# John-Ragland/pygenray

Measured on AMD Instinct MI355X. Metric: ray-steps/sec (whole node), 1e5-ray Munk fan to 1000 km; eigenray wall-clock, higher is better.
Workload: dtype f64

## Files before the change

pygenray_amd/csrc/pgr_crmath.h:

```cpp
#ifndef PGR_CRMATH_H
#define PGR_CRMATH_H

#ifdef PGR_CR_HOST
#include <math.h>
#define PGR_CR_FN static inline
#define PGR_CR_RARE(c) (__builtin_expect((c), 0))
#define PGR_CR_TABLE(type, name, n) static const type name[n]
static inline float pgr_cr_seed_log2f(float x) { return log2f(x); }
static inline float pgr_cr_seed_exp2f(float x) { return exp2f(x); }
static inline double pgr_cr_seed_asin(double x) { return asin(x); }
static inline double pgr_cr_fallback_sin(double x) { return sin(x); }
static inline double pgr_cr_fallback_pow(double x, double y) { return pow(x, y); }
#else
#define PGR_CR_FN __device__ __forceinline__
#define PGR_CR_RARE(c) (__builtin_expect(__builtin_amdgcn_ballot_w64(c) != 0ull, 0))
#define PGR_CR_TABLE(type, name, n) __device__ const type name[n]
__device__ __forceinline__ float pgr_cr_seed_log2f(float x) { return __builtin_amdgcn_logf(x); }
__device__ __forceinline__ float pgr_cr_seed_exp2f(float x) { return __builtin_amdgcn_exp2f(x); }
__device__ __forceinline__ double pgr_cr_seed_asin(double x) { return asin(x); }
__device__ __forceinline__ double pgr_cr_fallback_sin(double x) { return sin(x); }
__device__ __forceinline__ double pgr_cr_fallback_pow(double x, double y) { return pow(x, y); }
#endif

PGR_CR_TABLE(double, pgr_cr_sincos_tab, 29 * 4) = {
    0x0.0p+0, 0x0.0p+0, 0x1.0000000000000p+0, 0x0.0p+0,
    0x1.ffeaaaeeee86fp-6, -0x1.cd406fb224ae2p-60, 0x1.ffc00155527d3p-1, -0x1.3b54492d89b5bp-55,
    0x1.ffaaaeeed4edbp-5, -0x1.2d16d32684b69p-59, 0x1.ff0015549f4d3p-1, 0x1.328387b99426fp-55,
    0x1.7f701032550e4p-4, 0x1.afc2d1800501ap-60, 0x1.fdc06bf7e6b9bp-1, 0x1.31902b535f8dbp-55,
    0x1.feaaeee86ee36p-4, -0x1.afcb2bcc6f03bp-59, 0x1.fc015527d5bd3p-1, 0x1.b68f35094efb8p-55,
    0x1.3eb312c5d66cbp-3, 0x1.47d666b66cb91p-57, 0x1.f9c340a7cc428p-1, 0x1.c5b6b063b7462p-55,
    0x1.7dc102fbaf2b5p-3, 0x1.5ab50e23c97c3p-59, 0x1.f706bdf9ece1cp-1, -0x1.698c80c36dcb4p-55,
    0x1.bc6f84edc6199p-3, 0x1.9c1a56a7b0cabp-57, 0x1.f3cc7c3b3d16ep-1, -0x1.21a3ad28a3494p-57,
    0x1.faaeed4f31577p-3, -0x1.15d88508e32b8p-57, 0x1.f01549f7deea1p-1, 0x1.d3c1e99e5cafdp-55,
    0x1.1c37d64c6b876p-2, 0x1.46076fe0dcff4p-56, 0x1.ebe214f76efa8p-1, -0x1.02f9f12ba543ep-55,
    0x1.3ad129769d3d8p-2, 0x1.03d550487839ap-63, 0x1.e733ea0193d40p-1, -0x1.6428b3546ce13p-55,
    0x1.591bc9fa2f597p-2, 0x1.7c74bac3fe0cbp-57, 0x1.e20bf49acd6c1p-1, -0x1.660aec7ef636bp-58,
    0x1.7710255764214p-2, -0x1.6ead7314bb6cep-57, 0x1.dc6b7eb995912p-1, 0x1.4b364776dcd35p-58,
    0x1.94a6be9f546c5p-2, -0x1.69ce13e683f58p-56, 0x1.d653f073e4040p-1, -0x1.76236434bec37p-55,
    0x1.b1d8305321617p-2, -0x1.ae242cb99f519p-56, 0x1.cfc6cfa52ad9fp-1, 0x1.8b5b5508f2a0dp-55,
    0x1.ce9d2e3d4a51fp-2, -0x1.2fc8a12dae298p-57, 0x1.c8c5bf8ce1a84p-1, 0x1.ab3d1a1590123p-56,
    0x1.eaee8744b05f0p-2, -0x1.789b43c9b027dp-58, 0x1.c1528065b7d50p-1, -0x1.892111312e828p-55,
    0x1.0362939c69955p-1, -0x1.2d8cd78397b01p-55, 0x1.b96eeef58840ep-1, 0x1.45a3cc78fade0p-58,
    0x1.110d0c4b69c3bp-1, 0x1.d918998809981p-55, 0x1.b11d04162a4c6p-1, 0x1.1dd561efbc0c2p-56,
    0x1.1e7343236574cp-1, 0x1.22a3fa4f41d5ap-56, 0x1.a85ed4373e02dp-1, 0x1.9be06385ec792p-57,
    0x1.2b91dea88421ep-1, -0x1.fa371db216ab0p-55, 0x1.9f368ed912f85p-1, -0x1.1d200c5791606p-55,
    0x1.386597456282bp-1, -0x1.10fada93b07a8p-56, 0x1.95a67e00cb1fdp-1, -0x1.0befda21f862dp-55,
    0x1.44eb381cf386bp-1, -0x1.3ed6c1e6a5505p-55, 0x1.8bb105a5dc900p-1, 0x1.863e03e9474c1p-55,
    0x1.511f9fd7b351cp-1, -0x1.5c0e861c48831p-55, 0x1.8158a31916d5dp-1, -0x1.de8b90b8228dep-57,
    0x1.5cffc16bf8f0dp-1, 0x1.96cb370eb578ap-55, 0x1.769fec655211fp-1, -0x1.827d5cf8c68c5p-57,
    0x1.6888a4e134b2fp-1, -0x1.6b7d37644d5e6p-55, 0x1.6b898fa9efb5dp-1, 0x1.15ac786ccf4b2p-56,
    0x1.73b7680dea578p-1, -0x1.2248306dc12a2p-56, 0x1.6018526f563dfp-1, 0x1.46ca5e0e432d0p-55,
    0x1.7e893f5037959p-1, 0x1.0eefbaa650c4cp-55, 0x1.544f10f592ca5p-1, -0x1.e7ae8e6c7a62fp-55,
    0x1.88fb7640b8da2p-1, -0x1.49987c11efaa3p-55, 0x1.4830bd7d4ceb3p-1, 0x1.df77ff20d5448p-55,
};
#define PGR_CR_PIO2_H 0x1.921fb54442d18p+0
#define PGR_CR_PIO2_L 0x1.1a62633145c07p-54
#define PGR_CR_PIO2_1 0x1.921fb54400000p+0
#define PGR_CR_PIO2_2 0x1.0b4611a626331p-34
#define PGR_CR_PIO2_3 0x1.1701b839a2520p-88
#define PGR_CR_2OPI 0x1.45f306dc9c883p-1
#define PGR_CR_S3_H -0x1.5555555555555p-3
#define PGR_CR_S3_L -0x1.5555555555555p-57
#define PGR_CR_S5_H 0x1.1111111111111p-7
#define PGR_CR_S5_L 0x1.1111111111111p-63
#define PGR_CR_S7_H -0x1.a01a01a01a01ap-13
#define PGR_CR_S7_L -0x1.a01a01a01a01ap-73
#define PGR_CR_C4_H 0x1.5555555555555p-5
#define PGR_CR_C4_L 0x1.5555555555555p-59
#define PGR_CR_C6_H -0x1.6c16c16c16c17p-10
#define PGR_CR_C6_L 0x1.f49f49f49f49fp-65
#define PGR_CR_S9 0x1.71de3a556c734p-19
#define PGR_CR_S11 -0x1.ae64567f544e4p-26
#define PGR_CR_C8 0x1.a01a01a01a01ap-16
#define PGR_CR_C10 -0x1.27e4fb7789f5cp-22
#define PGR_CR_C12 0x1.1eed8eff8d898p-29
#define PGR_CR_POW_KLN2 -0x1.1be9bff2e94bfp-57

PGR_CR_FN double pgr_cr_newton5(double x, double y, const double fifth)
{
    const double y2 = y * y, y4 = y2 * y2, y5 = y4 * y;
    const double e = __builtin_fma(-x, y5, 1.0);
    return __builtin_fma(y * fifth, e, y);
}
PGR_CR_FN double pgr_cr_log2_slow(double x)
{
    union { double d; unsigned long long u; } v;
    v.d = x;
    int E = (int)((v.u >> 52) & 0x7ff) - 1023;
    v.u = (v.u & 0x000fffffffffffffULL) | 0x3ff0000000000000ULL;
    double m = v.d;
    if (m > 0x1.6a09e667f3bcdp+0) { m *= 0.5; E += 1; }
    const double z = (m - 1.0) / (m + 1.0), w = z * z;
    double p = 1.0 / 19.0;
    p = __builtin_fma(p, w, 1.0 / 17.0); p = __builtin_fma(p, w, 1.0 / 15.0); p = __builtin_fma(p, w, 1.0 / 13.0);
    p = __builtin_fma(p, w, 1.0 / 11.0); p = __builtin_fma(p, w, 1.0 / 9.0); p = __builtin_fma(p, w, 1.0 / 7.0);
    p = __builtin_fma(p, w, 1.0 / 5.0); p = __builtin_fma(p, w, 1.0 / 3.0); p = __builtin_fma(p, w, 1.0);
    return __builtin_fma(2.0 * z * p, 0x1.71547652b82fep+0, (double)E);
}
#define PGR_CR_ZIV_K 0x1.ffff8p-55
PGR_CR_FN int pgr_cr_rounding_uncertain(double res, double r)
{
#ifdef PGR_CR_HOST
    int e;
    (void)frexp(r, &e);
    const double thr = ldexp(PGR_CR_ZIV_K, e);
#else
    const double thr = __builtin_ldexp(PGR_CR_ZIV_K, __builtin_amdgcn_frexp_exp(r));
#endif
    return __builtin_fabs(res) > thr;
}
PGR_CR_FN double pgr_cr_pow_m02_slow(double x, double y, const double fifth, const double kln2)
{
    y = pgr_cr_newton5(x, y, fifth);
    const double ah = y * y, al = __builtin_fma(y, y, -ah);
    const double bh = ah * ah, bl = __builtin_fma(ah, al + al, __builtin_fma(ah, ah, -bh));
    const double ch = bh * y, cl = __builtin_fma(bl, y, __builtin_fma(bh, y, -ch));
    const double dh = ch * x, dl = __builtin_fma(cl, x, __builtin_fma(ch, x, -dh));
    const double rho = (1.0 - dh) - dl;
    const double u = __builtin_fma(pgr_cr_log2_slow(x), kln2, rho * fifth);
    return __builtin_fma(y, u, y);
}
PGR_CR_FN double pgr_cr_pow_m02_k(double x, const double fifth, const double kln2)
{
    const float lf = pgr_cr_seed_log2f((float)x);
    double y = (double)pgr_cr_seed_exp2f(-0.2f * lf);
    y = pgr_cr_newton5(x, y, fifth);
    const double ah = y * y, al = __builtin_fma(y, y, -ah);
    const double bh = ah * ah, bl = __builtin_fma(ah, al + al, __builtin_fma(ah, ah, -bh));
    const double ch = bh * y, cl = __builtin_fma(bl, y, __builtin_fma(bh, y, -ch));
    const double dh = ch * x, dl = __builtin_fma(cl, x, __builtin_fma(ch, x, -dh));
    const double rho = (1.0 - dh) - dl;
    const double r5 = rho * fifth;
    const double u = __builtin_fma((double)lf, kln2, __builtin_fma(-2.0 * r5, r5, r5));
    double r = __builtin_fma(y, u, y);
#ifndef PGR_POW_NO_ZIV
    if (PGR_CR_RARE(pgr_cr_rounding_uncertain(__builtin_fma(y, u, -(r - y)), r)))
        r = pgr_cr_pow_m02_slow(x, y, fifth, kln2);
#endif
    return r;
}
PGR_CR_FN double pgr_cr_pow_m02(double x) { return pgr_cr_pow_m02_k(x, 0.2, PGR_CR_POW_KLN2); }

PGR_CR_FN double pgr_cr_pow_p02_eval(double x, double w, double lg, double* approx, double* corr)
{
    const double ah = w * w, al = __builtin_fma(w, w, -ah);
    const double bh = ah * ah, bl = __builtin_fma(ah, al + al, __builtin_fma(ah, ah, -bh));
    const double ch = bh * w, cl = __builtin_fma(bl, w, __builtin_fma(bh, w, -ch));
    const double dh = ch * x, dl = __builtin_fma(cl, x, __builtin_fma(ch, x, -dh));
    const double rho = (1.0 - dh) - dl;
    const double rh = bh * x, rl = __builtin_fma(bl, x, __builtin_fma(bh, x, -rh));
    const double u = __builtin_fma(-lg, PGR_CR_POW_KLN2, rho * 0.8);
    *approx = rh;
    *corr = __builtin_fma(rh, u, rl);
    return rh + *corr;
}
PGR_CR_FN double pgr_cr_pow_p02(double x)
{
    if (!(x > 0x1.0p-60 && x < 0x1.0p+60)) return pgr_cr_fallback_pow(x, 0.2);
    const float lf = pgr_cr_seed_log2f((float)x);
    double w = (double)pgr_cr_seed_exp2f(-0.2f * lf);
    w = pgr_cr_newton5(x, pgr_cr_newton5(x, w, 0.2), 0.2);
    double approx, corr;
    double r = pgr_cr_pow_p02_eval(x, w, (double)lf, &approx, &corr);
#ifndef PGR_POW_NO_ZIV
    if (PGR_CR_RARE(pgr_cr_rounding_uncertain((approx - r) + corr, r)))
        r = pgr_cr_pow_p02_eval(x, w, pgr_cr_log2_slow(x), &approx, &corr);
#endif
    return r;
}

struct pgr_dd {
    double h, l;
};
PGR_CR_FN struct pgr_dd pgr_dd_fast_two_sum(double a, double b)
{
    struct pgr_dd r;
    r.h = a + b;
    r.l = b - (r.h - a);
    return r;
}
PGR_CR_FN struct pgr_dd pgr_dd_two_sum(double a, double b)
{
    struct pgr_dd r;
    r.h = a + b;
    const double bb = r.h - a;
    r.l = (a - (r.h - bb)) + (b - bb);
    return r;
}
PGR_CR_FN struct pgr_dd pgr_dd_mul(struct pgr_dd a, struct pgr_dd b)
{
    const double p = a.h * b.h;
    double e = __builtin_fma(a.h, b.h, -p);
    e = __builtin_fma(a.h, b.l, e);
    e = __builtin_fma(a.l, b.h, e);
    return pgr_dd_fast_two_sum(p, e);
}
PGR_CR_FN struct pgr_dd pgr_dd_add(struct pgr_dd a, struct pgr_dd b)
{
    const struct pgr_dd s = pgr_dd_two_sum(a.h, b.h);
    return pgr_dd_fast_two_sum(s.h, s.l + (a.l + b.l));
}
PGR_CR_FN struct pgr_dd pgr_dd_make(double h, double l)
{
    struct pgr_dd r;
    r.h = h;
    r.l = l;
    return r;
}

PGR_CR_FN void pgr_dd_sincos_x(struct pgr_dd y, struct pgr_dd* s_out, struct pgr_dd* c_out, const int c_plain)
{
    const double jr = __builtin_rint(y.h * 32.0);
    const struct pgr_dd d = pgr_dd_fast_two_sum(y.h - jr * 0.03125, y.l);
    const struct pgr_dd z = pgr_dd_mul(d, d);
    struct pgr_dd t = pgr_dd_two_sum(PGR_CR_S7_H, z.h * __builtin_fma(z.h, PGR_CR_S11, PGR_CR_S9));
    t.l += PGR_CR_S7_L;
    t = pgr_dd_add(pgr_dd_make(PGR_CR_S5_H, PGR_CR_S5_L), pgr_dd_mul(z, t));
    t = pgr_dd_add(pgr_dd_make(PGR_CR_S3_H, PGR_CR_S3_L), pgr_dd_mul(z, t));
    t = pgr_dd_mul(z, t);
    {
        const struct pgr_dd o = pgr_dd_fast_two_sum(1.0, t.h);
        t = pgr_dd_fast_two_sum(o.h, o.l + t.l);
    }
    const struct pgr_dd sd = pgr_dd_mul(d, t);
    struct pgr_dd u = pgr_dd_two_sum(
        PGR_CR_C6_H, z.h * __builtin_fma(z.h, __builtin_fma(z.h, PGR_CR_C12, PGR_CR_C10), PGR_CR_C8));
    u.l += PGR_CR_C6_L;
    u = pgr_dd_add(pgr_dd_make(PGR_CR_C4_H, PGR_CR_C4_L), pgr_dd_mul(z, u));
    u = pgr_dd_mul(z, u);
    {
        const struct pgr_dd o = pgr_dd_fast_two_sum(-0.5, u.h);
        u = pgr_dd_fast_two_sum(o.h, o.l + u.l);
    }
    u = pgr_dd_mul(z, u);
    {
        const struct pgr_dd o = pgr_dd_fast_two_sum(1.0, u.h);
        u = pgr_dd_fast_two_sum(o.h, o.l + u.l);
    }
    const struct pgr_dd cd = u;
    if (jr == 0.0) {
        *s_out = sd;
        *c_out = cd;
        return;
    }
    const int j = (int)__builtin_fabs(jr);
    const double sg = jr < 0.0 ? -1.0 : 1.0;
    const double* q = pgr_cr_sincos_tab + 4 * (j > 28 ? 28 : j);
    const struct pgr_dd sj = pgr_dd_make(sg * q[0], sg * q[1]), cj = pgr_dd_make(q[2], q[3]);
    *s_out = pgr_dd_add(pgr_dd_mul(sj, cd), pgr_dd_mul(cj, sd));
    if (c_plain) {
        *c_out = pgr_dd_make(cj.h * cd.h - sj.h * sd.h, 0.0);
        return;
    }
    const struct pgr_dd m = pgr_dd_mul(sj, sd);
    *c_out = pgr_dd_add(pgr_dd_mul(cj, cd), pgr_dd_make(-m.h, -m.l));
}
PGR_CR_FN void pgr_dd_sincos(struct pgr_dd y, struct pgr_dd* s_out, struct pgr_dd* c_out)
{
    pgr_dd_sincos_x(y, s_out, c_out, 0);
}

PGR_CR_FN double pgr_cr_sin(double x)
{
    if (x == 0.0) return x;
    if (!(__builtin_fabs(x) <= 6.5)) return pgr_cr_fallback_sin(x);
    const double kd = __builtin_rint(x * PGR_CR_2OPI);
    const double t = __builtin_fma(-kd, PGR_CR_PIO2_1, x);
    const double p = kd * PGR_CR_PIO2_2, pe = __builtin_fma(kd, PGR_CR_PIO2_2, -p);
    struct pgr_dd y = pgr_dd_two_sum(t, -p);
    y = pgr_dd_fast_two_sum(y.h, y.l - __builtin_fma(kd, PGR_CR_PIO2_3, pe));
    struct pgr_dd s, c;
    pgr_dd_sincos(y, &s, &c);
    const int n = ((int)kd) & 3;
    const double r = (n & 1) ? c.h : s.h;
    return (n & 2) ? -r : r;
}

PGR_CR_FN struct pgr_dd pgr_cr_asin_dd(double v)
{
    const double a = __builtin_fabs(v);
    if (!(a <= 1.0)) return pgr_dd_make(pgr_cr_seed_asin(v), 0.0);
    if (a == 0.0) return pgr_dd_make(v, 0.0);
    struct pgr_dd r, s, c;
    if (a <= 0.75) {
        const double a0 = pgr_cr_seed_asin(a);
        pgr_dd_sincos_x(pgr_dd_make(a0, 0.0), &s, &c, 1);
        r = pgr_dd_fast_two_sum(a0, ((a - s.h) - s.l) / c.h);
    } else {
        const double m = 1.0 - a;
        const struct pgr_dd n = pgr_dd_two_sum(1.0, a);
        const double ph = m * n.h, pl = __builtin_fma(m, n.l, __builtin_fma(m, n.h, -ph));
        const double wh = __builtin_sqrt(ph);
        struct pgr_dd b = pgr_dd_make(0.0, 0.0);
        if (wh > 0.0) {
            const double wl = (__builtin_fma(-wh, wh, ph) + pl) / (wh + wh);
            const double b0 = pgr_cr_seed_asin(wh);
            pgr_dd_sincos_x(pgr_dd_make(b0, 0.0), &s, &c, 1);
            b = pgr_dd_fast_two_sum(b0, (((wh - s.h) - s.l) + wl) / c.h);
        }
        const struct pgr_dd q = pgr_dd_two_sum(PGR_CR_PIO2_H, -b.h);
        r = pgr_dd_fast_two_sum(q.h, q.l + (PGR_CR_PIO2_L - b.l));
    }
    return v < 0.0 ? pgr_dd_make(-r.h, -r.l) : r;
}
PGR_CR_FN double pgr_cr_asin(double v) { return pgr_cr_asin_dd(v).h; }

PGR_CR_FN double pgr_cr_sin_near_minus_asin(double x, double v, struct pgr_dd A)
{
    const struct pgr_dd t = pgr_dd_two_sum(x, A.h);
    const double d = t.h + (t.l + A.l);
    if (!(__builtin_fabs(d) <= 0x1.0p-40 * __builtin_fabs(A.h)) || !(__builtin_fabs(v) < 0.999)) return pgr_cr_sin(x);
    const double w = __builtin_sqrt(__builtin_fma(-v, v, 1.0)) * d;
    return -v + w;
}

#endif
```

pygenray_amd/csrc/pgr_fan_kernel.h:

```cpp
#ifndef PGR_FAN_KERNEL_H
#define PGR_FAN_KERNEL_H

template <bool LDS_TAB, int ZM, int SAVE, bool PERSIST, bool LOG = false>
__global__ void __launch_bounds__(512)
pgr_fan_kernel(const EnvDev* __restrict__ env_p, typename FanKernelArgs<LOG>::type a)
{
    const EnvDev& env = *env_p;
    extern __shared__ double2 lds_tab[];
    double* const lds_after_tab = (double*)(lds_tab + (LDS_TAB ? env.nz : 0));
    double* const lds_z = lds_after_tab;
    unsigned short* const lds_zb = (unsigned short*)(lds_z + env.nz);
    if (LDS_TAB) {
        for (int j = threadIdx.x; j < env.nz; j += blockDim.x) lds_tab[j] = env.tab[j];
    }
    if (ZM == 2 || ZM == 3 || ZM == 5) {
        for (int j = threadIdx.x; j < env.nz; j += blockDim.x) lds_z[j] = env.zin[j];
        if (ZM == 2) for (int j = threadIdx.x; j < env.zb_B; j += blockDim.x) lds_zb[j] = env.zbucket[j];
    }
    double* const lds_bx = (a.bathy_lds_off >= 0) ? (double*)((char*)lds_tab + a.bathy_lds_off) : nullptr;
    if (lds_bx) {
        for (int j = threadIdx.x; j < env.nb; j += blockDim.x) {
            lds_bx[j] = env.depth_ranges[j];
            lds_bx[env.nb + j] = env.depths[j];
        }
    }
    const int wv = threadIdx.x >> 6;
    const int n_cw = (int)(blockDim.x >> 6);
    __syncthreads();
    const Ctx<LDS_TAB, ZM> C(env, lds_tab, lds_z, lds_zb, lds_bx);
    C.declare_span(a.x0, a.x1);
    bool first_packet = true;
    for (;;) {
    const char __attribute__((address_space(4))) * kq_p =
        (const char __attribute__((address_space(4))) *)__builtin_amdgcn_kernarg_segment_ptr();
    if (PERSIST) asm volatile("" : "+s"(kq_p));
    const FanArgs __attribute__((address_space(4))) & aq = *(const FanArgs __attribute__((address_space(4))) *)(kq_p + kFanArgsKernargOffset);
    int* const wave_queue = PERSIST ? aq.wave_queue : nullptr;
    const int* const q_map = PERSIST ? aq.wave_map : a.wave_map;
    const int64_t q_N = PERSIST ? aq.N : a.N, q_stride_ray = PERSIST ? aq.stride_ray : a.stride_ray;
    const double* const q_y0 = PERSIST ? aq.y0 : a.y0;
    const uint32_t q_flags = PERSIST ? aq.flags : a.flags;
    int64_t gwave = (int64_t)wv * gridDim.x + blockIdx.x;
    if (q_map) {
        int slot = blockIdx.x * n_cw + wv;
        if (PERSIST && wave_queue) {
            const int n_tail = aq.n_queue_tail, n_head = aq.n_queue - n_tail;
            if (first_packet && wv >= 4 && n_tail) {
                slot = aq.n_queue - 1 - ((int)blockIdx.x * 4 + (wv - 4));
            } else {
                int got = 0;
                if ((threadIdx.x & 63) == 0) got = atomicAdd(wave_queue, 1);
                slot = __builtin_amdgcn_readfirstlane(got);
                if (slot >= n_head) break;
            }
            first_packet = false;
        }
        int m = q_map[slot];
        gwave = (m < 0) ? -1 : (m & 0x0fffffff);
        int prio = __builtin_amdgcn_readfirstlane((m < 0) ? 0 : ((m >> 28) & 3));
        if (prio == 3) __builtin_amdgcn_s_setprio(3);
        else if (prio == 2) __builtin_amdgcn_s_setprio(2);
        else if (prio == 1) __builtin_amdgcn_s_setprio(1);
        else if (PERSIST) __builtin_amdgcn_s_setprio(0);
    }
    if (PERSIST) C.reset_range_cache();
#ifdef PGR_WAVE_TIMES
    const unsigned wt_start = (unsigned)__builtin_amdgcn_s_memrealtime();
#endif
    const int64_t ray = gwave * 64 + (threadIdx.x & 63);
    const bool valid = (gwave >= 0) && (ray < q_N);
    double SAFETY = 0.9, MIN_FACTOR = 0.2, MAX_FACTOR = 10,
           SQRT3 = 1.7320508075688772, INV_SQRT3 = 0.57735026918962584,
           POW_FIFTH = 0.2, POW_KLN2 = PGR_CR_POW_KLN2;
    const double rtol = a.rtol, atol = a.atol, t_bound = a.x1;
    const int S = a.S;
    constexpr bool save = (SAVE != 0);
    const bool exact_samples = (SAVE == 2) && (a.flags & PGR_EXACT_SAMPLES) != 0;
    const int attempt_limit = (int)((4 * a.max_steps + 4096 < 0x3fffffff) ? 4 * a.max_steps + 4096 : 0x3fffffff);
    const unsigned long long sgn = (a.flags & PGR_STORED_SIGN) ? 0x8000000000000000ULL : 0ULL;
#define SGN(v) __longlong_as_double(__double_as_longlong(v) ^ (long long)sgn)
    SaveGrid G;
    G.r = a.r_save; G.x0 = a.x0; G.x1 = a.x1; G.step = a.save_step;
    G.S = S; G.formula = (SAVE == 1 || SAVE == 3) ? 1 : a.save_formula;

    double t = a.x0, y0 = 0, y1 = 0, y2 = 0;
    if (valid) {
        y0 = q_y0[3 * ray + 0];
        y1 = q_y0[3 * ray + 1];
        y2 = q_y0[3 * ray + 2];
    }
    double f0 = 0, f1 = 0, f2 = 0, h_abs = 0;
    unsigned g = 0;
    int status = valid ? RUNNING : PGR_RAY_OK;
    if (valid && (q_flags & PGR_SKIP_NAN_Y0) && (y2 != y2)) status = PGR_RAY_SKIPPED;
    bool need_init = true, rejected = false, parked = false;
    int nb = 0, ns = 0, n_steps = 0, n_rej = 0;
    int jnext = 0;
    double rnext = 0;
    double pk_tnew = 0;
    unsigned pk_active = 0;
    int waited = 0;
    int trips = 0, services = 0, fallbacks = 0;
    const double min_step_bound = 10 * 0x1p-52 * fmax(fabs(a.x0), fabs(a.x1)) + 1e-300;
    const int max_steps32 = (int)(a.max_steps < 0x7fffffff ? a.max_steps : 0x7fffffff);
    const int guard_limit = (max_steps32 < attempt_limit ? max_steps32 : attempt_limit);
#if defined(PGR_TIMING) || defined(PGR_SVC_TIMING)
    unsigned tacc[24];
    for (int k = 0; k < 24; k++) tacc[k] = 0;
    unsigned tprev = (unsigned)clock64();
#endif
    const int64_t out_off = ray * q_stride_ray;
#define Tp (a.T + out_off)
#define Zp (a.Z + out_off)
#define Pp (a.P + out_off)
    constexpr bool BLK = (SAVE == 3);
    static_assert(!(BLK && LDS_TAB), "the blocked sample layout is instantiated for the HBM-table kernels only");
    double* const blk = (double*)((char*)lds_tab + (BLK ? a.blk_lds_off : 0)) + (wv * 768 + (int)(threadIdx.x & 63));
    auto blk_flush = [&](int jb) __attribute__((always_inline)) {
        const int64_t o = ((int64_t)jb * a.N + ray) * 4;
        typedef double d2 __attribute__((ext_vector_type(2)));
        const d2 t0 = {blk[0], blk[64]}, t1 = {blk[128], blk[192]};
        const d2 z0 = {blk[256], blk[320]}, z1 = {blk[384], blk[448]};
        const d2 p0 = {blk[512], blk[576]}, p1 = {blk[640], blk[704]};
        __builtin_nontemporal_store(t0, (d2*)(a.T + o)); __builtin_nontemporal_store(t1, (d2*)(a.T + o + 2));
        __builtin_nontemporal_store(z0, (d2*)(a.Z + o)); __builtin_nontemporal_store(z1, (d2*)(a.Z + o + 2));
        __builtin_nontemporal_store(p0, (d2*)(a.P + o)); __builtin_nontemporal_store(p1, (d2*)(a.P + o + 2));
    };
    auto emit_sample = [&](int j, double vt, double vz, double vp) __attribute__((always_inline)) {
        if (BLK) {
            double* const e = blk + (j & 3) * 64;
            e[0] = vt; e[256] = vz; e[512] = vp;
            if ((j & 3) == 3) blk_flush(j >> 2);
            return;
        }
        const int64_t o = (int64_t)j * a.stride_smp;
        if (LDS_TAB) { Tp[o] = vt; Zp[o] = vz; Pp[o] = vp; }
        else {
            __builtin_nontemporal_store(vt, &Tp[o]);
            __builtin_nontemporal_store(vz, &Zp[o]);
            __builtin_nontemporal_store(vp, &Pp[o]);
        }
    };

#define PGR_VCONST(n) double v##n = n; asm volatile("" : "+v"(v##n))
    PGR_VCONST(A21);
    PGR_VCONST(A31);
    PGR_VCONST(A32);
    PGR_VCONST(A41);
    PGR_VCONST(A42);
    PGR_VCONST(A43);
    PGR_VCONST(A51);
    PGR_VCONST(A52);
    PGR_VCONST(A53);
    PGR_VCONST(A54);
    PGR_VCONST(A61);
    PGR_VCONST(A62);
    PGR_VCONST(A63);
    PGR_VCONST(A64);
    PGR_VCONST(A65);
    PGR_VCONST(B1);
    PGR_VCONST(B3);
    PGR_VCONST(B4);
    PGR_VCONST(B5);
    PGR_VCONST(B6);
    PGR_VCONST(E1);
    PGR_VCONST(E3);
    PGR_VCONST(E4);
    PGR_VCONST(E5);
    PGR_VCONST(E6);
    PGR_VCONST(E7);
#undef PGR_VCONST
    constexpr bool PIN_P = (SAVE != 0 && ZM != 0 && ZM != 3);
#define PGR_VCONST_IF(c, n) double v##n = n; if (c) asm volatile("" : "+v"(v##n))
    PGR_VCONST_IF(PIN_P, P11);
    PGR_VCONST_IF(PIN_P, P12);
    PGR_VCONST_IF(PIN_P, P13);
    PGR_VCONST_IF(PIN_P, P31);
    PGR_VCONST_IF(PIN_P, P32);
    PGR_VCONST_IF(PIN_P, P33);
    PGR_VCONST_IF(PIN_P, P41);
    PGR_VCONST_IF(PIN_P, P42);
    PGR_VCONST_IF(PIN_P, P43);
    PGR_VCONST_IF(PIN_P, P51);
    PGR_VCONST_IF(PIN_P, P52);
    PGR_VCONST_IF(PIN_P, P53);
    PGR_VCONST_IF(PIN_P, P61);
    PGR_VCONST_IF(PIN_P, P62);
    PGR_VCONST_IF(PIN_P, P63);
    PGR_VCONST_IF(PIN_P, P71);
    PGR_VCONST_IF(PIN_P, P72);
    PGR_VCONST_IF(PIN_P, P73);
#undef PGR_VCONST_IF
    constexpr bool PIN_LITERALS = (SAVE == 0 || ZM == 3);
    if (PIN_LITERALS) {
#define PGR_PIN(x) asm volatile("" : "+v"(x))
        PGR_PIN(C.k_c2); PGR_PIN(C.k_c3); PGR_PIN(C.k_c4); PGR_PIN(C.k_c5); PGR_PIN(C.k_tiny); PGR_PIN(C.k_vert);
        PGR_PIN(SAFETY); PGR_PIN(MIN_FACTOR); PGR_PIN(MAX_FACTOR);
        PGR_PIN(SQRT3); PGR_PIN(INV_SQRT3);
        PGR_PIN(POW_FIFTH); PGR_PIN(POW_KLN2);
#undef PGR_PIN
    }
    constexpr int PIN_ZC = (SAVE != 0 ? 2 : 1);
    if (ZM == 5 && PIN_ZC >= 1) {
        asm volatile("" : "+v"(C.h_zc_g2));
        asm volatile("" : "+v"(C.h_zc_s1));
    }
    if (ZM == 5 && PIN_ZC >= 2) {
        asm volatile("" : "+v"(C.h_zc_g0));
        asm volatile("" : "+v"(C.h_zc_g1));
        asm volatile("" : "+v"(C.h_zc_g3));
        asm volatile("" : "+v"(C.h_zc_s0));
        asm volatile("" : "+v"(C.h_zc_s2));
    }
    constexpr bool KEEPK = !(ZM == 5 && SAVE != 0);
    double k30 = 0, k31 = 0, k32 = 0, k40 = 0, k41 = 0, k42 = 0, k50 = 0, k51 = 0, k52 = 0, k60 = 0, k61 = 0, k62 = 0,
           k70 = 0, k71 = 0, k72 = 0;
    do {
        bool run, pend;
        unsigned long long pm;
        do {
        trips++;
        PGR_STAMP(0);
        if (status == RUNNING && !parked && !need_init) {
            bool too_small = false;
            if (__builtin_expect(ballot64(h_abs < min_step_bound) != 0, 0)) {
                double min_step = min_step_of(t);
                if (!rejected && h_abs < min_step) h_abs = min_step;
                too_small = h_abs < min_step;
                if (too_small) status = PGR_RAY_STEP_TOO_SMALL;
            }
            double h = h_abs;
            double t_new = t + h;
            if ((t_new - t_bound) > 0) t_new = t_bound;
            h = t_new - t;
            h_abs = fabs(h);

            PGR_RK_STAGES_BODY(t, h);
            double sc0 = atol + fmax(fabs(y0), fabs(n0)) * rtol;
            double sc1 = atol + fmax(fabs(y1), fabs(n1)) * rtol;
            double sc2 = atol + fmax(fabs(y2), fabs(n2)) * rtol;
            double er0 = fdiv(es0 * h, sc0);
            double er1 = fdiv(es1 * h, sc1);
            double er2 = fdiv(es2 * h, sc2);
            double error_norm = rms3(er0, er1, er2, SQRT3, INV_SQRT3);
            PGR_STAMP(15);

            const bool accepted = !too_small && (error_norm < 1);
            const bool reject = !too_small && !accepted;
            const double pw = SAFETY * pow_m02(error_norm, POW_FIFTH, POW_KLN2);
            double fac_acc = (pw < MAX_FACTOR) ? pw : MAX_FACTOR;
            fac_acc = (rejected && !(fac_acc < 1)) ? 1.0 : fac_acc;
            const double fac_rej = (pw > MIN_FACTOR) ? pw : MIN_FACTOR;
            h_abs = h_abs * (accepted ? fac_acc : fac_rej);
            rejected = reject;
            n_rej += reject ? 1 : 0;
            const bool guards_due = trips > guard_limit;
            if (__builtin_expect(guards_due, 0)) {
                const bool over = (n_rej + n_steps) > attempt_limit;
                status = (reject & over) ? PGR_RAY_MAX_STEPS : status;
                trips = trips < 0x7f000000 ? trips : 0x7f000000;
            }
            PGR_STAMP(16);

            if (accepted) {
                n_steps++;
                unsigned g_new = C.events(t_new, n1, n2, c_new);
                PGR_STAMP(17);
                unsigned up = (~g) & g_new, down = g & (~g_new);
                unsigned active = (up & 3u) | ((up | down) & 12u);
                g = g_new;
                bool want_samples = save && (jnext < S - 1) && (rnext <= t_new);
                const bool scipy_order = exact_samples || (rnext < t);
                Dense D;
                if (active) {
                    parked = true;
                    pk_active = active;
                    pk_tnew = t_new;
                } else {
                    if (want_samples) {
                        if (scipy_order) {
                            PGR_FORM_Q();
                            while (jnext < S - 1 && rnext <= t_new) {
                                double o0, o1, o2;
                                D.eval(t, y0, y1, y2, rnext, o0, o1, o2);
                                emit_sample(jnext, o0, SGN(o1), SGN(o2));
                                jnext++;
                                rnext = G.at(jnext);
                            }
                        } else {
                            const double inv_h = frcp_seed(h);
#define PGR_KSUM(k1, k3, k4, k5, k6, k7)                                                          \
    __builtin_fma(k1, b1, __builtin_fma(k3, b3, __builtin_fma(k4, b4, __builtin_fma(k5, b5,      \
                  __builtin_fma(k6, b6, (k7) * b7)))))
#define PGR_SAMPLE_LOOP(NEXT)                                                                     \
    while (jnext < S - 1 && rnext <= t_new) {                                                     \
        const double xi = (rnext - t) * inv_h, x2 = xi * xi;                                      \
        const double b1 = xi * __builtin_fma(xi, __builtin_fma(xi, __builtin_fma(xi, vP13, vP12), vP11), P10); \
        const double b3 = x2 * __builtin_fma(xi, __builtin_fma(xi, vP33, vP32), vP31);               \
        const double b4 = x2 * __builtin_fma(xi, __builtin_fma(xi, vP43, vP42), vP41);               \
        const double b5 = x2 * __builtin_fma(xi, __builtin_fma(xi, vP53, vP52), vP51);               \
        const double b6 = x2 * __builtin_fma(xi, __builtin_fma(xi, vP63, vP62), vP61);               \
        const double b7 = x2 * __builtin_fma(xi, __builtin_fma(xi, vP73, vP72), vP71);               \
        emit_sample(jnext, __builtin_fma(h, PGR_KSUM(f0, k30, k40, k50, k60, k70), y0),            \
                    SGN(__builtin_fma(h, PGR_KSUM(f1, k31, k41, k51, k61, k71), y1)),               \
                    SGN(__builtin_fma(h, PGR_KSUM(f2, k32, k42, k52, k62, k72), y2)));              \
        jnext++;                                                                                  \
        rnext = NEXT;                                                                             \
    }
                            if (SAVE == 1 || SAVE == 3 || G.formula) { PGR_SAMPLE_LOOP(grid_at(G.x0, G.step, jnext)) }
                            else { PGR_SAMPLE_LOOP(G.r[jnext]) }
#undef PGR_SAMPLE_LOOP
#undef PGR_KSUM
                        }
                    }
                    t = t_new; y0 = n0; y1 = n1; y2 = n2;
                    f0 = k70; f1 = k71; f2 = k72;
                    status = ((t - t_bound) >= 0) ? PGR_RAY_OK : status;
                    if (__builtin_expect(guards_due, 0))
                        status = (status == RUNNING && n_steps > max_steps32) ? PGR_RAY_MAX_STEPS : status;
                }
                PGR_STAMP(18);
            }
        }
        PGR_STAMP(19);
        run = (status == RUNNING);
        pend = run && (parked || need_init);
        pm = ballot64(pend);
        } while (pm == 0 && ballot64(run) != 0);
        asm volatile("" : "+s"(pm));
        if (pm) {
            waited++;
            const bool nobody_steps = ballot64(run && !pend) == 0;
            if (__popcll(pm) >= a.park_lanes || waited > a.park_trips || nobody_steps) {
                waited = 0;
                services++;
                PGR_SSTAMP(23);
                const EnvDev* es_p = env_p;
                asm volatile("" : "+s"(es_p));
                const EnvDev& es = *es_p;
                const char __attribute__((address_space(4))) * ks_p =
                    (const char __attribute__((address_space(4))) *)__builtin_amdgcn_kernarg_segment_ptr();
                asm volatile("" : "+s"(ks_p));
                const FanArgs __attribute__((address_space(4))) & as = *(const FanArgs __attribute__((address_space(4))) *)(ks_p + kFanArgsKernargOffset);
                const double svc_c_lo = es.c_lo, svc_c_hi = es.c_hi;
                if (pend && parked) {
                    parked = false;
                    const unsigned active = pk_active;
                    const double t_new = pk_tnew, h = t_new - t;
                    Dense D;
                    PGR_SSTAMP(0);
                    if (KEEPK) {
                        PGR_FORM_Q();
                    } else {
                        PGR_RK_STAGES(t, h);
                        (void)n0; (void)c_new; (void)es0; (void)es1; (void)es2;
                        PGR_FORM_Q();
                    }
                    PGR_SSTAMP(1);
                    int ev = -1;
                    double best = 0;
                    const bool with_bbox = (active == 9u);
                    const unsigned act = with_bbox ? 1u : active;
                    if ((a.flags & PGR_EXACT_BISECTION) == 0 && (act == 1u || act == 2u)) {
                        const bool bottom = (act == 2u);
                        const double q0 = D.q[1][0], q1 = D.q[1][1], q2 = D.q[1][2], q3 = D.q[1][3];
                        double bs = 0, be = 0;
                        int cell_s = 0, cell_e = 0;
                        if (bottom) { bs = C.bathy(t, cell_s); be = C.bathy(t_new, cell_e); }
                        double zb = y1 + h * (q0 + q1 + q2 + q3);
                        double Fa = bottom ? (y1 - bs) : y1;
                        double Fb = bottom ? (zb - be) : zb;
                        bool pre = bottom ? (Fa <= 0 && Fb > 0) : (Fa >= 0 && Fb < 0);
                        double xa = t, xb = t_new;
                        bool live = false;
                        const bool any_bottom = ballot64(bottom) != 0;
                        const bool chord = ballot64(bottom && cell_s != cell_e) == 0;
                        PGR_SSTAMP(2);
                        if (pre) {
                            const double bslope = bottom ? (be - bs) : 0.0;
                            double lo = 0.0, hi = 1.0;
                            double sN = fdiv(Fa, Fa - Fb);
                            double dFs = 0;
                            for (int it = 0; it < 16; it++) {
                                double zs = y1 + h * (sN * (q0 + sN * (q1 + sN * (q2 + sN * q3))));
                                double dz = h * (q0 + sN * (2 * q1 + sN * (3 * q2 + sN * 4 * q3)));
                                double F = zs, dF = dz;
                                if (any_bottom) {
                                    double bq;
                                    if (chord) bq = bs + sN * bslope;
                                    else bq = C.bathy(t + sN * h);
                                    F = bottom ? zs - bq : zs;
                                    dF = bottom ? dz - bslope : dz;
                                }
                                dFs = dF;
                                bool crossed = bottom ? (F > 0) : (F < 0);
                                if (crossed) hi = sN; else lo = sN;
                                double sn = sN - F * frcp_seed(dF);
                                if (!(sn >= lo && sn <= hi)) sn = 0.5 * (lo + hi);
                                double ds = fabs(sn - sN);
                                sN = sn;
                                if (it >= 2 && ballot64(ds * h >= 1e-12 * (1.0 + fabs(t))) == 0) break;
                            }
                            PGR_SSTAMP(3);
                            const double xs = t + sN * h;
                            const double E = 2 * DBL_EPSILON * (fabs(y1) + fabs(h) * (fabs(q0) + fabs(q1) + fabs(q2) + fabs(q3)) +
                                                                (bottom ? fabs(bs) + fabs(be) : 0.0));
                            const double nu = 4 * E * fabs(h) / fabs(dFs);
                            xa = fmax(nextafter(xs - nu, -INFINITY), t);
                            xb = fmin(nextafter(xs + nu, INFINITY), t_new);
#define PGR_TRUE_EVENT(X_, FIRED_, BBOX_)                                                                        \
    do {                                                                                                         \
        const double xx_ = fdiv((X_) - t, D.h);                                                                  \
        const double e1_ = xx_, e2_ = e1_ * xx_, e3_ = e2_ * xx_, e4_ = e3_ * xx_;                               \
        const double z_ = D.h * (D.q[1][0] * e1_ + D.q[1][1] * e2_ + D.q[1][2] * e3_ + D.q[1][3] * e4_) + y1;   \
        const double pz_ = D.h * (D.q[2][0] * e1_ + D.q[2][1] * e2_ + D.q[2][2] * e3_ + D.q[2][3] * e4_) + y2;  \
                            \
        double pc_ = pz_;                                                                                        \
        if (ballot64(!((svc_c_lo > 0) & (fabs(pz_) * svc_c_hi < 1.0))) != 0) {                                    \
            double c_, cp_;                                                                                      \
            C.lookup((X_), z_, c_, cp_);                                                                         \
            pc_ = pz_ * c_;                                                                                      \
        }                                                                                                        \
        const double bd_ = any_bottom ? C.bathy(X_) : 0.0;                                                       \
        FIRED_ = bottom ? ((pc_ > 0) & (pc_ <= 1.0) & (z_ > bd_)) : ((z_ < 0) & (pc_ < 0) & (pc_ >= -1.0));       \
        BBOX_ = (z_ > C.h_zhi_tol) | (z_ < C.h_zlo_tol) | ((X_) < es.rlo_tol) | ((X_) > es.rhi_tol);             \
    } while (0)
                            bool ga, gb, bbox_a, bbox_b;
                            PGR_TRUE_EVENT(xa, ga, bbox_a);
                            PGR_TRUE_EVENT(xb, gb, bbox_b);
                            (void)bbox_a;
                            live = (xa < xb) && !ga && gb && !(with_bbox && bbox_b);
                            PGR_SSTAMP(4);
                            {
                                const double x1 = next_up(xa), x2 = next_up(x1), x3 = next_up(x2);
                                const int m = !live ? 3 : (x1 >= xb) ? 0 : (x2 >= xb) ? 1 : (x3 >= xb) ? 2 : 3;
                                bool g1 = true, g2 = true, bbox_q;
                                if (ballot64(m == 1 || m == 2) != 0) { PGR_TRUE_EVENT(x1, g1, bbox_q); }
                                if (ballot64(m == 2) != 0) { PGR_TRUE_EVENT(x2, g2, bbox_q); }
                                (void)bbox_q;
                                g1 = (m == 1 || m == 2) ? g1 : true;
                                g2 = (m == 2) ? g2 : true;
                                if (m <= 2 && (g2 || !g1)) {
                                    const double nxa = g1 ? xa : (g2 ? x1 : x2);
                                    xb = g1 ? x1 : (g2 ? x2 : xb);
                                    xa = nxa;
                                }
                            }
                            PGR_SSTAMP(5);
                        }
                        const double xtol = 4 * DBL_EPSILON, brtol = 4 * DBL_EPSILON;
                        double cur = t_new, xblk = t;
                        bool fcur = true;
                        {
                            const double dmax = (xtol + brtol * fmax(fabs(t), fabs(t_new))) / 2;
                            const bool sterbenz = (t > 0) ? (t_new <= 2 * t) : ((t_new < 0) && (t >= 2 * t_new));
                            int n1 = (live && sterbenz) ? ilogb(h) - ilogb(dmax) - 3 : (live ? 0 : 90);
                            n1 = min(max(n1, 0), 90);
                            {
                                int m = 0;
#pragma unroll
                                for (int bit = 64; bit > 0; bit >>= 1)
                                    if (ballot64(n1 < m + bit) == 0) m += bit;
                                n1 = m;
                            }
                            double plo = t, phi = t_new;
                            bool lastc = true;
#pragma unroll 4
                            for (int k = 0; k < n1; k++) {
                                const double nw = __builtin_fma(phi - plo, 0.5, plo);
                                const bool ge = (nw >= xb), le = (nw <= xa);
                                phi = ge ? nw : phi;
                                plo = le ? nw : plo;
                                lastc = ge | (lastc & !le);
                            }
                            if (n1 > 0) { cur = lastc ? phi : plo; xblk = lastc ? plo : phi; fcur = lastc; }
                        }
                        PGR_SSTAMP(6);
                        double fcv = fcur ? 1.0 : 0.0;
                        bool done = !live;
                        for (int it = 0; it < 200; it++) {
                            const double dlt = (xtol + brtol * fabs(cur)) / 2;
                            const double sbis = (xblk - cur) / 2;
                            done = !live | (fabs(sbis) < dlt);
                            if (ballot64(!done) == 0) break;
                            const double nw = (fabs(sbis) > dlt) ? cur + sbis : cur + (sbis > 0 ? dlt : -dlt);
                            const bool inside = !done & (nw > xa) & (nw < xb);
                            double fnv = (nw >= xb) ? 1.0 : 0.0;
                            if (ballot64(inside) != 0) {
                                bool fired, bbox_q;
                                PGR_TRUE_EVENT(nw, fired, bbox_q);
                                (void)bbox_q;
                                fnv = inside ? (fired ? 1.0 : 0.0) : fnv;
                            }
                            xblk = (!done & (fnv != fcv)) ? cur : xblk;
                            cur = done ? cur : nw;
                            fcv = done ? fcv : fnv;
                        }
                        if (live && done) { best = cur; ev = bottom ? 1 : 0; }
                        PGR_SSTAMP(7);
                    }
                    if (ev < 0) {
                        fallbacks++;
                        const double xtol = 4 * DBL_EPSILON, brtol = 4 * DBL_EPSILON;
                        for (int k = 0; k < 4; k++) {
                            if (!(active & (1u << k))) continue;
                            double xpre = t, xcur = t_new, xblk = 0;
                            double ez0, ez1, ez2, ec, ecp;
                            D.eval(t, y0, y1, y2, xpre, ez0, ez1, ez2);
                            C.lookup(xpre, ez1, ec, ecp);
                            bool fpre = (C.events(xpre, ez1, ez2, ec) >> k) & 1u;
                            D.eval(t, y0, y1, y2, xcur, ez0, ez1, ez2);
                            C.lookup(xcur, ez1, ec, ecp);
                            bool fcur = (C.events(xcur, ez1, ez2, ec) >> k) & 1u;
                            if (fpre == fcur) { status = PGR_RAY_EVENT_ERROR; break; }
                            for (int it = 0; it < 100; it++) {
                                if (fpre != fcur) xblk = xpre;
                                double delta = (xtol + brtol * fabs(xcur)) / 2;
                                double sbis = (xblk - xcur) / 2;
                                if (fabs(sbis) < delta) break;
                                xpre = xcur;
                                fpre = fcur;
                                if (fabs(sbis) > delta) xcur += sbis;
                                else xcur += (sbis > 0 ? delta : -delta);
                                D.eval(t, y0, y1, y2, xcur, ez0, ez1, ez2);
                                C.lookup(xcur, ez1, ec, ecp);
                                fcur = (C.events(xcur, ez1, ez2, ec) >> k) & 1u;
                            }
                            if (ev < 0 || xcur < best) { best = xcur; ev = k; }
                        }
                    }
                    PGR_SSTAMP(8);
                    if (status == RUNNING) {
                        const double t_end = best;
                        if (save) {
                            while (jnext < S - 1 && rnext <= t_end) {
                                double o0, o1, o2;
                                D.eval(t, y0, y1, y2, rnext, o0, o1, o2);
                                emit_sample(jnext, o0, SGN(o1), SGN(o2));
                                jnext++;
                                rnext = G.at(jnext);
                            }
                        }
                        PGR_SSTAMP(9);
                        double r0, r1, r2;
                        D.eval(t, y0, y1, y2, t_end, r0, r1, r2);
                        t = t_end; y0 = r0; y1 = r1; y2 = r2;
                        PGR_SSTAMP(10);
                        if (ev == 2) status = PGR_RAY_VERTICAL;
                        else if (ev == 3) status = PGR_RAY_BBOX;
                        else {
                            double c, cp;
                            C.lookup(t, y1, c, cp);
                            const double pc_b = y2 * c;
                            const struct pgr_dd A_b = pgr_cr_asin_dd(pc_b);
                            double theta = A_b.h * (180.0 / M_PI);
                            double theta_b;
                            PGR_SSTAMP(11);
                            if (ev == 0) {
                                theta_b = -theta;
                                ns++;
                            } else {
                                const double* xr = es.depth_ranges;
                                if (!(t >= xr[0] && t <= xr[es.nb - 1])) {
                                    status = PGR_RAY_BETA_RANGE;
                                    theta_b = 0;
                                } else {
                                    double beta = 0.0;
                                    if (!es.beta_zero) {
                                        int i;
                                        double xi;
                                        if (es.b_uniform) {
                                            i = cell_uniform(t, es.b0, es.db, es.inv_db, es.nb);
                                            xi = grid_at(es.b0, es.db, i);
                                        } else {
                                            i = cell_search(t, xr, es.nb);
                                            xi = xr[i];
                                        }
                                        double u = t - xi;
                                        const double* q = es.pp + 4 * i;
                                        beta = q[0] + u * (q[1] + u * (q[2] + u * q[3]));
                                    }
                                    theta_b = 2 * beta - theta;
                                    nb++;
                                }
                            }
                            PGR_SSTAMP(12);
                            if (status == RUNNING) {
                                if ((as.flags & PGR_TERMINATE_BACKWARDS) && (fabs(theta_b) > 90))
                                    status = PGR_RAY_BACKWARD;
                                else {
                                    y2 = fdiv(pgr_cr_sin_near_minus_asin(theta_b * (M_PI / 180.0), pc_b, A_b), c);
                                    need_init = true;
                                    if constexpr (LOG) {
                                        const FanArgsLog __attribute__((address_space(4))) & al =
                                            *(const FanArgsLog __attribute__((address_space(4))) *)(ks_p + kFanArgsKernargOffset);
                                        const int e = nb + ns - 1;
                                        if (e < al.log_K) {
                                            const int64_t o = (int64_t)e * as.N + ray;
                                            al.log_x[o] = t;
                                            al.log_p[o] = SGN(y2);
                                            al.log_k[o] = (signed char)ev;
                                        }
                                    }
                                    if (!(t < t_bound)) status = PGR_RAY_OK;
                                    else if (n_steps > max_steps32) status = PGR_RAY_MAX_STEPS;
                                }
                            }
                        }
                    }
                }
                PGR_SSTAMP(13);
                if (status == RUNNING && need_init) {
                    double c;
                    C.rhs(t, y1, y2, f0, f1, f2, c);
                    double interval = fabs(t_bound - t);
                    double s0 = atol + fabs(y0) * rtol, s1 = atol + fabs(y1) * rtol,
                           s2 = atol + fabs(y2) * rtol;
                    double d0 = rms3(fdiv(y0, s0), fdiv(y1, s1), fdiv(y2, s2));
                    double d1 = rms3(fdiv(f0, s0), fdiv(f1, s1), fdiv(f2, s2));
                    double h0 = (d0 < 1e-5 || d1 < 1e-5) ? 1e-6 : fdiv(0.01 * d0, d1);
                    if (!(h0 < interval)) h0 = interval;
                    PGR_SSTAMP(14);
                    double e0, e1, e2, cdummy;
                    C.rhs(t + h0 * 1.0, y1 + h0 * 1.0 * f1, y2 + h0 * 1.0 * f2, e0, e1, e2, cdummy);
                    double d2 = fdiv(rms3(fdiv(e0 - f0, s0), fdiv(e1 - f1, s1), fdiv(e2 - f2, s2)), h0);
                    double h1;
                    if (d1 <= 1e-15 && d2 <= 1e-15) {
                        h1 = h0 * 1e-3;
                        if (!(h1 > 1e-6)) h1 = 1e-6;
                    } else {
                        h1 = pgr_cr_pow_p02(fdiv(0.01, (d2 > d1) ? d2 : d1));
                    }
                    PGR_SSTAMP(15);
                    h_abs = 100 * h0;
                    if (h1 < h_abs) h_abs = h1;
                    if (interval < h_abs) h_abs = interval;
                    g = C.events(t, y1, y2, c);
                    rejected = false;
                    need_init = false;
                    if (save) {
                        jnext = G.nearest(t, as.inv_dsave);
                        rnext = G.at(jnext);
                    }
                    PGR_SSTAMP(16);
                }
                PGR_SSTAMP(17);
            }
        }
    } while (ballot64(status == RUNNING) != 0);

    if (valid) {
        bool ok = (status == PGR_RAY_OK);
        double nan = __longlong_as_double(0x7ff8000000000000LL);
        typedef const FanArgs __attribute__((address_space(4))) * KArgs;
        const char __attribute__((address_space(4))) * kp =
            (const char __attribute__((address_space(4))) *)__builtin_amdgcn_kernarg_segment_ptr();
        asm volatile("" : "+s"(kp));
        const FanArgs __attribute__((address_space(4))) & a = *(KArgs)(kp + kFanArgsKernargOffset);
        if (BLK) {
            if (ok) {
                const int last = (S - 1) & 3;
                double* const e = blk + last * 64;
                e[0] = y0; e[256] = SGN(y1); e[512] = SGN(y2);
                for (int k = last + 1; k < 4; k++) { blk[k * 64] = nan; blk[256 + k * 64] = nan; blk[512 + k * 64] = nan; }
                blk_flush((S - 1) >> 2);
            } else {
                for (int k = 0; k < 12; k++) blk[k * 64] = nan;
                for (int jb = 0; jb < (S + 3) / 4; jb++) blk_flush(jb);
            }
        } else if (save) {
            if (ok) {
                Tp[(int64_t)(S - 1) * a.stride_smp] = y0;
                Zp[(int64_t)(S - 1) * a.stride_smp] = SGN(y1);
                Pp[(int64_t)(S - 1) * a.stride_smp] = SGN(y2);
            } else {
                for (int j = 0; j < S; j++) {
                    Tp[(int64_t)j * a.stride_smp] = nan;
                    Zp[(int64_t)j * a.stride_smp] = nan;
                    Pp[(int64_t)j * a.stride_smp] = nan;
                }
            }
        }
        if (a.end_state) {
            if (a.flags & PGR_PACKED_END) {
                double* rec = a.end_state + 5 * ray;
                rec[0] = ok ? y0 : nan; rec[1] = ok ? y1 : nan; rec[2] = ok ? y2 : nan;
                int* ir = (int*)(rec + 3);
                ir[0] = nb; ir[1] = ns; ir[2] = status; ir[3] = 1;
            } else {
                a.end_state[3 * ray + 0] = ok ? y0 : nan;
                a.end_state[3 * ray + 1] = ok ? y1 : nan;
                a.end_state[3 * ray + 2] = ok ? y2 : nan;
            }
        }
        a.n_bott[ray] = nb;
        a.n_surf[ray] = ns;
        a.status[ray] = status;
        if (a.n_steps) a.n_steps[ray] = n_steps;
#if defined(PGR_TIMING) || defined(PGR_SVC_TIMING)
        if ((threadIdx.x & 63) < 24) {
            unsigned v = 0;
            for (int k = 0; k < 24; k++) v = ((threadIdx.x & 63) == k) ? tacc[k] : v;
            n_rej = (int)v;
        }
#endif
#ifdef PGR_WAVE_TIMES
        if (a.flags & PGR_DEBUG_TRIPS) {
            const int ln = (int)(threadIdx.x & 63);
            const unsigned wt_end = (unsigned)__builtin_amdgcn_s_memrealtime();
            const unsigned hw_id = __builtin_amdgcn_s_getreg((4 ) | (0 << 6) | (31 << 11));
            const unsigned xcc_id = __builtin_amdgcn_s_getreg((20 ) | (0 << 6) | (31 << 11));
            fallbacks = ln == 3 ? (int)wt_start : ln == 4 ? (int)wt_end : ln == 5 ? (int)hw_id : ln == 6 ? (int)xcc_id
                        : ln == 7 ? (int)blockIdx.x : fallbacks;
        }
#endif
        if (a.n_rej) a.n_rej[ray] = (a.flags & PGR_DEBUG_TRIPS) ? (((threadIdx.x & 63) == 0) ? trips : (((threadIdx.x & 63) == 1) ? services : fallbacks)) : n_rej;
    }
    if (!PERSIST || !wave_queue) break;
    }
#undef Tp
#undef Zp
#undef Pp
#undef SGN
}

#endif
```

Measured before the change: 25.91 billion.

## Batch service-path scalar loads and make bisection loops branchless with sign masks

The service path now loads environment and kernarg scalars in one batch through constant address space and pins them in scalar registers, for the LDS_TAB/ZM==4 specialization. The Newton event solve runs three unconditional steps before its first wave vote. The halving and bisection loops become branchless sign-mask selects, unrolled by eight, with fewer ballots per iteration. The fallback path is now gated by a wave-wide ballot. The aim is to cut scalar-memory latency, divergence and vote overhead in the rare parked-ray service, at the cost of extra work when rays converge early and higher register pressure.

```diff
diff --git a/pygenray_amd/csrc/pgr_crmath.h b/pygenray_amd/csrc/pgr_crmath.h
--- a/pygenray_amd/csrc/pgr_crmath.h
+++ b/pygenray_amd/csrc/pgr_crmath.h
@@ -21,6 +21,21 @@
 __device__ __forceinline__ double pgr_cr_fallback_sin(double x) { return sin(x); }
 __device__ __forceinline__ double pgr_cr_fallback_pow(double x, double y) { return pow(x, y); }
 #endif
+
+PGR_CR_FN int pgr_sign_mask(double d)
+{
+    union { double d; unsigned long long u; } v;
+    v.d = d;
+    return (int)(v.u >> 32) >> 31;
+}
+PGR_CR_FN double pgr_mask_select(int m, double a, double b)
+{
+    union { double d; unsigned long long u; } va, vb;
+    const unsigned long long mm = ((unsigned long long)(unsigned)m << 32) | (unsigned)m;
+    va.d = a; vb.d = b;
+    va.u = (va.u & mm) | (vb.u & ~mm);
+    return va.d;
+}
 
 PGR_CR_TABLE(double, pgr_cr_sincos_tab, 29 * 4) = {
     0x0.0p+0, 0x0.0p+0, 0x1.0000000000000p+0, 0x0.0p+0,
diff --git a/pygenray_amd/csrc/pgr_fan_kernel.h b/pygenray_amd/csrc/pgr_fan_kernel.h
--- a/pygenray_amd/csrc/pgr_fan_kernel.h
+++ b/pygenray_amd/csrc/pgr_fan_kernel.h
@@ -335,14 +335,27 @@
                 waited = 0;
                 services++;
                 PGR_SSTAMP(23);
-                const EnvDev* es_p = env_p;
+                typedef const EnvDev __attribute__((address_space(4))) EnvConst;
+                EnvConst* es_p = (EnvConst*)env_p;
                 asm volatile("" : "+s"(es_p));
-                const EnvDev& es = *es_p;
+                EnvConst& es = *es_p;
                 const char __attribute__((address_space(4))) * ks_p =
                     (const char __attribute__((address_space(4))) *)__builtin_amdgcn_kernarg_segment_ptr();
                 asm volatile("" : "+s"(ks_p));
                 const FanArgs __attribute__((address_space(4))) & as = *(const FanArgs __attribute__((address_space(4))) *)(ks_p + kFanArgsKernargOffset);
-                const double svc_c_lo = es.c_lo, svc_c_hi = es.c_hi;
+                constexpr bool SVC_BATCH = LDS_TAB && ZM == 4;
+                double svc_c_lo = es.c_lo, svc_c_hi = es.c_hi;
+                double svc_rlo_tol = 0, svc_rhi_tol = 0, svc_b_xlo = 0, svc_b_xhi = 0, svc_inv_dsave = 0;
+                int svc_beta_zero = 0;
+                uint32_t svc_flags = 0;
+                if (SVC_BATCH) {
+                    svc_rlo_tol = es.rlo_tol; svc_rhi_tol = es.rhi_tol;
+                    svc_b_xlo = es.b_xlo; svc_b_xhi = es.b_xhi;
+                    svc_beta_zero = es.beta_zero;
+                    svc_flags = as.flags;
+                    if (save) svc_inv_dsave = as.inv_dsave;
+                }
+#define PGR_SVC(batched_, lazy_) (SVC_BATCH ? (batched_) : (lazy_))
                 if (pend && parked) {
                     parked = false;
                     const unsigned active = pk_active;
@@ -356,6 +369,9 @@
                         (void)n0; (void)c_new; (void)es0; (void)es1; (void)es2;
                         PGR_FORM_Q();
                     }
+                    if (SVC_BATCH)
+                        asm volatile("" : "+s"(svc_c_lo), "+s"(svc_c_hi), "+s"(svc_rlo_tol), "+s"(svc_rhi_tol), "+s"(svc_b_xlo),
+                                          "+s"(svc_b_xhi), "+s"(svc_beta_zero), "+s"(svc_flags));
                     PGR_SSTAMP(1);
                     int ev = -1;
                     double best = 0;
@@ -381,7 +397,8 @@
                             double lo = 0.0, hi = 1.0;
                             double sN = fdiv(Fa, Fa - Fb);
                             double dFs = 0;
-                            for (int it = 0; it < 16; it++) {
+                            double ds = 0;
+                            auto newton_step = [&]() __attribute__((always_inline)) {
                                 double zs = y1 + h * (sN * (q0 + sN * (q1 + sN * (q2 + sN * q3))));
                                 double dz = h * (q0 + sN * (2 * q1 + sN * (3 * q2 + sN * 4 * q3)));
                                 double F = zs, dF = dz;
@@ -397,9 +414,17 @@
                                 if (crossed) hi = sN; else lo = sN;
                                 double sn = sN - F * frcp_seed(dF);
                                 if (!(sn >= lo && sn <= hi)) sn = 0.5 * (lo + hi);
-                                double ds = fabs(sn - sN);
+                                ds = fabs(sn - sN);
                                 sN = sn;
-                                if (it >= 2 && ballot64(ds * h >= 1e-12 * (1.0 + fabs(t))) == 0) break;
+                            };
+                            newton_step();
+                            newton_step();
+                            newton_step();
+                            if (__builtin_expect(ballot64(ds * h >= 1e-12 * (1.0 + fabs(t))) != 0, 0)) {
+                                for (int it = 3; it < 16; it++) {
+                                    newton_step();
+                                    if (ballot64(ds * h >= 1e-12 * (1.0 + fabs(t))) == 0) break;
+                                }
                             }
                             PGR_SSTAMP(3);
                             const double xs = t + sN * h;
@@ -416,14 +441,15 @@
         const double pz_ = D.h * (D.q[2][0] * e1_ + D.q[2][1] * e2_ + D.q[2][2] * e3_ + D.q[2][3] * e4_) + y2;  \
                             \
         double pc_ = pz_;                                                                                        \
-        if (ballot64(!((svc_c_lo > 0) & (fabs(pz_) * svc_c_hi < 1.0))) != 0) {                                    \
+        if (__builtin_expect(ballot64(!((svc_c_lo > 0) & (fabs(pz_) * svc_c_hi < 1.0))) != 0, 0)) {               \
             double c_, cp_;                                                                                      \
             C.lookup((X_), z_, c_, cp_);                                                                         \
             pc_ = pz_ * c_;                                                                                      \
         }                                                                                                        \
         const double bd_ = any_bottom ? C.bathy(X_) : 0.0;                                                       \
         FIRED_ = bottom ? ((pc_ > 0) & (pc_ <= 1.0) & (z_ > bd_)) : ((z_ < 0) & (pc_ < 0) & (pc_ >= -1.0));       \
-        BBOX_ = (z_ > C.h_zhi_tol) | (z_ < C.h_zlo_tol) | ((X_) < es.rlo_tol) | ((X_) > es.rhi_tol);             \
+        BBOX_ = (z_ > C.h_zhi_tol) | (z_ < C.h_zlo_tol) | ((X_) < PGR_SVC(svc_rlo_tol, es.rlo_tol)) |             \
+                ((X_) > PGR_SVC(svc_rhi_tol, es.rhi_tol));                                                       \
     } while (0)
                             bool ga, gb, bbox_a, bbox_b;
                             PGR_TRUE_EVENT(xa, ga, bbox_a);
@@ -450,7 +476,7 @@
                         }
                         const double xtol = 4 * DBL_EPSILON, brtol = 4 * DBL_EPSILON;
                         double cur = t_new, xblk = t;
-                        bool fcur = true;
+                        int fcm = -1;
                         {
                             const double dmax = (xtol + brtol * fmax(fabs(t), fabs(t_new))) / 2;
                             const bool sterbenz = (t > 0) ? (t_new <= 2 * t) : ((t_new < 0) && (t >= 2 * t_new));
@@ -464,42 +490,62 @@
                                 n1 = m;
                             }
                             double plo = t, phi = t_new;
-                            bool lastc = true;
-#pragma unroll 4
-                            for (int k = 0; k < n1; k++) {
+                            int lastm = -1;
+                            auto halving = [&]() __attribute__((always_inline)) {
                                 const double nw = __builtin_fma(phi - plo, 0.5, plo);
-                                const bool ge = (nw >= xb), le = (nw <= xa);
-                                phi = ge ? nw : phi;
-                                plo = le ? nw : plo;
-                                lastc = ge | (lastc & !le);
-                            }
-                            if (n1 > 0) { cur = lastc ? phi : plo; xblk = lastc ? plo : phi; fcur = lastc; }
+                                const int m_lt = pgr_sign_mask(nw - xb);
+                                const int m_gt = pgr_sign_mask(xa - nw);
+                                phi = pgr_mask_select(m_lt, phi, nw);
+                                plo = pgr_mask_select(m_gt, plo, nw);
+                                lastm = ~m_lt | (lastm & m_gt);
+                            };
+                            int k = n1;
+#pragma unroll 1
+                            for (; k >= 8; k -= 8) {
+                                halving(); halving(); halving(); halving(); halving(); halving(); halving(); halving();
+                            }
+                            if (k & 4) { halving(); halving(); halving(); halving(); }
+                            if (k & 2) { halving(); halving(); }
+                            if (k & 1) halving();
+                            cur = pgr_mask_select(lastm, phi, plo);
+                            xblk = pgr_mask_select(lastm, plo, phi);
+                            fcm = lastm;
                         }
                         PGR_SSTAMP(6);
-                        double fcv = fcur ? 1.0 : 0.0;
-                        bool done = !live;
+                        const int m_live = live ? -1 : 0;
+                        int m_done = ~m_live, m_in = 0;
+                        double nw = cur;
                         for (int it = 0; it < 200; it++) {
-                            const double dlt = (xtol + brtol * fabs(cur)) / 2;
-                            const double sbis = (xblk - cur) / 2;
-                            done = !live | (fabs(sbis) < dlt);
-                            if (ballot64(!done) == 0) break;
-                            const double nw = (fabs(sbis) > dlt) ? cur + sbis : cur + (sbis > 0 ? dlt : -dlt);
-                            const bool inside = !done & (nw > xa) & (nw < xb);
-                            double fnv = (nw >= xb) ? 1.0 : 0.0;
-                            if (ballot64(inside) != 0) {
+#pragma unroll
+                            for (int u = 0; u < 8; u++) {
+                                const double dlt = (xtol + brtol * fabs(cur)) / 2;
+                                const double sbis = (xblk - cur) / 2;
+                                const double asb = fabs(sbis);
+                                m_done = ~m_live | pgr_sign_mask(asb - dlt);
+                                nw = cur + pgr_mask_select(pgr_sign_mask(dlt - asb), sbis, __builtin_copysign(dlt, sbis));
+                                const int m_ltb = pgr_sign_mask(nw - xb);
+                                m_in = ~m_done & pgr_sign_mask(xa - nw) & m_ltb;
+                                const int m_go = ~(m_done | m_in);
+                                if (ballot64(m_go != 0) == 0) break;
+                                xblk = pgr_mask_select(m_go & (~m_ltb ^ fcm), cur, xblk);
+                                cur = pgr_mask_select(m_go, nw, cur);
+                                fcm = (~m_ltb & m_go) | (fcm & ~m_go);
+                            }
+                            if (__builtin_expect(ballot64(m_in != 0) != 0, 0)) {
                                 bool fired, bbox_q;
                                 PGR_TRUE_EVENT(nw, fired, bbox_q);
                                 (void)bbox_q;
-                                fnv = inside ? (fired ? 1.0 : 0.0) : fnv;
-                            }
-                            xblk = (!done & (fnv != fcv)) ? cur : xblk;
-                            cur = done ? cur : nw;
-                            fcv = done ? fcv : fnv;
+                                const int m_f = fired ? -1 : 0;
+                                xblk = pgr_mask_select(m_in & (m_f ^ fcm), cur, xblk);
+                                cur = pgr_mask_select(m_in, nw, cur);
+                                fcm = (m_f & m_in) | (fcm & ~m_in);
+                            } else if (ballot64(m_done == 0) == 0) break;
                         }
+                        const bool done = m_done != 0;
                         if (live && done) { best = cur; ev = bottom ? 1 : 0; }
                         PGR_SSTAMP(7);
                     }
-                    if (ev < 0) {
+                    if (__builtin_expect(ballot64(ev < 0) != 0, 0) && ev < 0) {
                         fallbacks++;
                         const double xtol = 4 * DBL_EPSILON, brtol = 4 * DBL_EPSILON;
                         for (int k = 0; k < 4; k++) {
@@ -561,12 +607,12 @@
                                 ns++;
                             } else {
                                 const double* xr = es.depth_ranges;
-                                if (!(t >= xr[0] && t <= xr[es.nb - 1])) {
+                                if (!(t >= PGR_SVC(svc_b_xlo, es.b_xlo) && t <= PGR_SVC(svc_b_xhi, es.b_xhi))) {
                                     status = PGR_RAY_BETA_RANGE;
                                     theta_b = 0;
                                 } else {
                                     double beta = 0.0;
-                                    if (!es.beta_zero) {
+                                    if (!PGR_SVC(svc_beta_zero, es.beta_zero)) {
                                         int i;
                                         double xi;
                                         if (es.b_uniform) {
@@ -586,7 +632,7 @@
                             }
                             PGR_SSTAMP(12);
                             if (status == RUNNING) {
-                                if ((as.flags & PGR_TERMINATE_BACKWARDS) && (fabs(theta_b) > 90))
+                                if ((PGR_SVC(svc_flags, as.flags) & PGR_TERMINATE_BACKWARDS) && (fabs(theta_b) > 90))
                                     status = PGR_RAY_BACKWARD;
                                 else {
                                     y2 = fdiv(pgr_cr_sin_near_minus_asin(theta_b * (M_PI / 180.0), pc_b, A_b), c);
@@ -610,6 +656,7 @@
                     }
                 }
                 PGR_SSTAMP(13);
+                if (save && SVC_BATCH) asm volatile("" : "+s"(svc_inv_dsave));
                 if (status == RUNNING && need_init) {
                     double c;
                     C.rhs(t, y1, y2, f0, f1, f2, c);
@@ -639,7 +686,7 @@
                     rejected = false;
                     need_init = false;
                     if (save) {
-                        jnext = G.nearest(t, as.inv_dsave);
+                        jnext = G.nearest(t, PGR_SVC(svc_inv_dsave, as.inv_dsave));
                         rnext = G.at(jnext);
                     }
                     PGR_SSTAMP(16);
@@ -718,6 +765,7 @@
     }
     if (!PERSIST || !wave_queue) break;
     }
+#undef PGR_SVC
 #undef Tp
 #undef Zp
 #undef Pp
```

Result: faster. 26.36 billion, median of 6 (+1.7%).
